# MikeIvanichev/norma

Hardware: AMD Instinct MI355X
Metric: audio-sec/wall-sec (xRT) distil-large-v3 fp16 b32 (higher is better)
Workload: dtype f16

## Files before the change

norma_amd/csrc/k_gemm.hip:

```cpp
#include <stdlib.h>

#include <atomic>

#include "mfma_tile128.h"

#define BM 128
#define BN 128
#define BK 64

__device__ __forceinline__ float gelu_tanh_f(float v) { return gelu_tanh_fast(v); }

__device__ __forceinline__ const half_t *a_row_ptr(const GemmParams &p, int m) {
    if (m >= p.M) m = p.M - 1;
    int b = nh_div(m, p.a_rpb, p.a_magic), r = m - b * p.a_rpb;
    return p.A + (long)b * p.a_bstride + (long)r * p.lda;
}

template <bool SWAP>
__device__ __forceinline__ void gemm_mainloop(const GemmParams &p, char *smem, int m0, int n0, f32x4 (&acc)[4][4]) {
    tile128_mainloop<SWAP>([&](int row) { return a_row_ptr(p, m0 + row); },
                           [&](int row) { return p.W + (long)(n0 + row) * p.K; }, p.K / BK, smem, acc);
}

__device__ __forceinline__ long out_row(const GemmParams &p, int m) {
    int b = nh_div(m, p.o_rpb, p.o_magic), r = m - b * p.o_rpb;
    return (long)b * p.o_bstride + r + p.o_off;
}

__global__ __launch_bounds__(256, 2) void gemm_f16_kernel(GemmParams p) {
    __shared__ __attribute__((aligned(16))) char smem[T128_LDS];
    const int ntn = p.N / BN, ntm = (p.M + BM - 1) / BM;
    const int bid = xcd_contiguous(blockIdx.x, ntn * ntm);
    const int tm = bid / ntn, tn = bid - tm * ntn;
    const int m0 = tm * BM, n0 = tn * BN;
    const int lane = threadIdx.x & 63, w = threadIdx.x >> 6;
    const int wm = w >> 1, wn = w & 1;
    const int fr = lane & 15, fq = lane >> 4;

    f32x4 acc[4][4];
#pragma unroll
    for (int i = 0; i < 4; i++)
#pragma unroll
        for (int j = 0; j < 4; j++) acc[i][j] = (f32x4){0.f, 0.f, 0.f, 0.f};

    const int seg = (p.epi == EPI_F16 || p.epi == EPI_GELU_F16) ? n0 / p.seg_n : 0;
    const bool vt = (p.epi == EPI_F16 && seg == p.vt_seg);
    if (vt) gemm_mainloop<false>(p, smem, m0, n0, acc);
    else gemm_mainloop<true>(p, smem, m0, n0, acc);

    if (vt) {
        half_t *dst = reinterpret_cast<half_t *>(seg == 0 ? p.out[0] : seg == 1 ? p.out[1] : p.out[2]);
#pragma unroll
        for (int i = 0; i < 4; i++) {
            int n = n0 + wn * 64 + 16 * i + fr;
            float bv = p.bias ? p.bias[n] : 0.f;
            int nl = n - seg * p.seg_n, h = nl >> 6, dh = nl & 63;
#pragma unroll
            for (int j = 0; j < 4; j++) {
                int m = m0 + wm * 64 + 16 * j + 4 * fq;
                if (m >= p.M) continue;
                int b = nh_div(m, p.S, p.s_magic), s = m - b * p.S;
                half_t *row = dst + ((long)(b * p.H + h) * NH_DH + dh) * NH_SP;
                if (s + 3 < p.S && m + 3 < p.M) {
                    half4 v = {(half_t)(acc[i][j][0] + bv), (half_t)(acc[i][j][1] + bv),
                               (half_t)(acc[i][j][2] + bv), (half_t)(acc[i][j][3] + bv)};
                    *reinterpret_cast<half4 *>(row + s) = v;
                } else {
                    for (int r = 0; r < 4; r++) {
                        int mm = m + r;
                        if (mm >= p.M) break;
                        int bb = nh_div(mm, p.S, p.s_magic), ss = mm - bb * p.S;
                        dst[((long)(bb * p.H + h) * NH_DH + dh) * NH_SP + ss] = (half_t)(acc[i][j][r] + bv);
                    }
                }
            }
        }
        return;
    }
    half_t *obase = reinterpret_cast<half_t *>(seg == 0 ? p.out[0] : seg == 1 ? p.out[1] : p.out[2]);
#pragma unroll
    for (int i = 0; i < 4; i++) {
        const int n = n0 + wn * 64 + 16 * i + 4 * fq;
        f32x4 bv = {0.f, 0.f, 0.f, 0.f};
        if (p.bias) bv = *reinterpret_cast<const f32x4 *>(p.bias + n);
#pragma unroll
        for (int j = 0; j < 4; j++) {
            const int m = m0 + wm * 64 + 16 * j + fr;
            if (m >= p.M) continue;
            f32x4 v = acc[i][j] + bv;
            if (p.epi == EPI_F16 || p.epi == EPI_GELU_F16) {
                if (p.epi == EPI_F16 && seg == 0 && p.seg0_scale != 0.f) v *= p.seg0_scale;
                if (p.epi == EPI_GELU_F16) {
                    v[0] = gelu_tanh_f(v[0]); v[1] = gelu_tanh_f(v[1]);
                    v[2] = gelu_tanh_f(v[2]); v[3] = gelu_tanh_f(v[3]);
                }
                const int nl = n - seg * p.seg_n;
                half_t *dst = p.head_major ? obase + (((long)nh_div(m, p.S, p.s_magic) * p.H + (nl >> 6)) * p.S + (m - nh_div(m, p.S, p.s_magic) * p.S)) * NH_DH + (nl & 63)
                                           : obase + out_row(p, m) * p.ldo + nl;
                half4 hv = {(half_t)v[0], (half_t)v[1], (half_t)v[2], (half_t)v[3]};
                *reinterpret_cast<half4 *>(dst) = hv;
            } else if (p.epi == EPI_RESID_F32) {
                float *dst = reinterpret_cast<float *>(p.out[0]) + (long)m * p.ldo + n;
                f32x4 x = *reinterpret_cast<const f32x4 *>(dst);
                *reinterpret_cast<f32x4 *>(dst) = x + v;
            } else {
                int s = m - nh_div(m, p.S, p.s_magic) * p.S;
                f32x4 pe = *reinterpret_cast<const f32x4 *>(p.pos + (long)s * p.N + n);
                f32x4 o = {gelu_tanh_f(v[0]) + pe[0], gelu_tanh_f(v[1]) + pe[1], gelu_tanh_f(v[2]) + pe[2],
                           gelu_tanh_f(v[3]) + pe[3]};
                *reinterpret_cast<f32x4 *>(reinterpret_cast<float *>(p.out[0]) + (long)m * p.ldo + n) = o;
            }
        }
    }
}

#define G2_BM 256
#define G2_BN 256
#define G2_GM 4
#define PP_BUF 65536
#define PP_HT 16384
#define PP_RING (2 * PP_BUF)
#define PP_EPI_PITCH 136
#define PP_EPI_WAVE (16 * PP_EPI_PITCH)
#define PP_BIAS (PP_RING + 8 * PP_EPI_WAVE)
#define PP_LDS (PP_BIAS + 2 * 1024)
#define PP_VT_OOB 0xf0000000u

struct PPSource { unsigned ag[2][2], wg[2][2]; };

__device__ __forceinline__ PPSource pp_source(const GemmParams &p, int m0, int n0) {
    int tid = threadIdx.x;
    asm volatile("" : "+v"(tid));
    const int lrow = tid >> 3;
    const int csrc = ((tid & 7) ^ ((lrow >> 1) & 7)) * 8;
    PPSource sg;
#pragma unroll
    for (int h = 0; h < 2; h++)
#pragma unroll
        for (int i = 0; i < 2; i++) {
            const unsigned m = (unsigned)min(m0 + i * 128 + h * 64 + lrow, p.M - 1), b = __umulhi(m, p.a_magic);
            sg.ag[h][i] = b * (unsigned)p.a_bstride + (m - b * (unsigned)p.a_rpb) * (unsigned)p.lda + csrc;
            const int l = lrow + 64 * i;
            sg.wg[h][i] = (unsigned)(n0 + (l >> 5) * 64 + h * 32 + (l & 31)) * (unsigned)p.K + csrc;
        }
    return sg;
}

__device__ __forceinline__ void pp_stage(const GemmParams &p, char *wbase, const PPSource &sg, int t, int which) {
    const int h = (which >> 1) & 1;
    const bool isB = which == 1 || which == 2;
    char *dst = wbase + (t & 1) * PP_BUF + (isB ? 2 * PP_HT : 0) + h * PP_HT;
    const unsigned ko = (unsigned)t * 64u;
    if (isB) {
        __builtin_amdgcn_global_load_lds((gbl_void *)(p.W + (size_t)(sg.wg[h][0] + ko)), (lds_void *)dst, 16, 0, 0);
        __builtin_amdgcn_global_load_lds((gbl_void *)(p.W + (size_t)(sg.wg[h][1] + ko)), (lds_void *)(dst + 8192), 16, 0, 0);
    } else {
        __builtin_amdgcn_global_load_lds((gbl_void *)(p.A + (size_t)(sg.ag[h][0] + ko)), (lds_void *)dst, 16, 0, 0);
        __builtin_amdgcn_global_load_lds((gbl_void *)(p.A + (size_t)(sg.ag[h][1] + ko)), (lds_void *)(dst + 8192), 16, 0, 0);
    }
}

__device__ __forceinline__ void pp_prologue(const GemmParams &p, char *wbase, const PPSource &sg) {
    pp_stage(p, wbase, sg, 0, 0); pp_stage(p, wbase, sg, 0, 1); pp_stage(p, wbase, sg, 0, 2); pp_stage(p, wbase, sg, 0, 3);
    pp_stage(p, wbase, sg, 1, 0); pp_stage(p, wbase, sg, 1, 1);
}

template <bool SWAP>
__device__ __forceinline__ void pp_main(const GemmParams &p, char *smem, char *wbase, const PPSource &sg, f32x4 (&acc)[8][4]) {
    const int lane = threadIdx.x & 63, w = threadIdx.x >> 6;
    const int wr = w >> 2, wc = w & 3;
    const int fr = lane & 15, fq = lane >> 4;
    const int nt = p.K >> 6;
    const int offA0 = (wr * 64 + fr) * 128 + ((fq ^ (fr >> 1)) << 4);
    const int offB0 = (wc * 32 + fr) * 128 + ((fq ^ (fr >> 1)) << 4);
    const char *const pa[2] = {smem + offA0, smem + (offA0 ^ 64)};
    const char *const pb[2] = {smem + offB0, smem + (offB0 ^ 64)};
    half8 fa[4][2], fb[4][2];

#define PP_PHASE(Q, BUF, WAIT, DO_ISSUE, ST)                                                                             \
    {                                                                                                                    \
        constexpr int tb_ = (BUF) * PP_BUF;                                                                              \
        if ((Q) == 0) {                                                                                                  \
            _Pragma("unroll") for (int j = 0; j < 2; j++) _Pragma("unroll") for (int ks = 0; ks < 2; ks++)             \
                fb[j][ks] = *reinterpret_cast<const half8 *>(pb[ks] + (tb_ + 2 * PP_HT + 2048 * j));                    \
            __builtin_amdgcn_sched_barrier(0);                                                                           \
            _Pragma("unroll") for (int i = 0; i < 4; i++) _Pragma("unroll") for (int ks = 0; ks < 2; ks++)             \
                fa[i][ks] = *reinterpret_cast<const half8 *>(pa[ks] + (tb_ + 2048 * i));                               \
        } else if ((Q) == 1) {                                                                                           \
            _Pragma("unroll") for (int j = 0; j < 2; j++) _Pragma("unroll") for (int ks = 0; ks < 2; ks++)             \
                fb[2 + j][ks] = *reinterpret_cast<const half8 *>(pb[ks] + (tb_ + 3 * PP_HT + 2048 * j));                \
        } else if ((Q) == 2) {                                                                                           \
            _Pragma("unroll") for (int i = 0; i < 4; i++) _Pragma("unroll") for (int ks = 0; ks < 2; ks++)             \
                fa[i][ks] = *reinterpret_cast<const half8 *>(pa[ks] + (tb_ + PP_HT + 2048 * i));                       \
        }                                                                                                                \
        __builtin_amdgcn_sched_barrier(0);                                                                               \
        if (DO_ISSUE) pp_stage(p, wbase, sg, (ST), (Q) == 2 ? 0 : (Q) == 3 ? 1 : (Q) == 0 ? 2 : 3);                     \
        if ((WAIT) == 8) asm volatile("s_waitcnt vmcnt(8)" ::: "memory");                                                \
        else if ((WAIT) == 4) asm volatile("s_waitcnt vmcnt(4)" ::: "memory");                                           \
        else if ((WAIT) == 2) asm volatile("s_waitcnt vmcnt(2)" ::: "memory");                                           \
        else if ((WAIT) == 0) asm volatile("s_waitcnt vmcnt(0)" ::: "memory");                                           \
        __builtin_amdgcn_s_barrier();                                                                                    \
        asm volatile("s_waitcnt lgkmcnt(0)" ::: "memory");                                                               \
        __builtin_amdgcn_sched_barrier(0);                                                                               \
        __builtin_amdgcn_s_setprio(1);                                                                                   \
        {                                                                                                                \
            constexpr int ib_ = ((Q) >= 2) ? 4 : 0, jb_ = ((Q) == 1 || (Q) == 2) ? 2 : 0;                                \
            _Pragma("unroll") for (int ks = 0; ks < 2; ks++) _Pragma("unroll") for (int i = 0; i < 4; i++)             \
                _Pragma("unroll") for (int j = 0; j < 2; j++) {                                                         \
                    if (SWAP) acc[ib_ + i][jb_ + j] = __builtin_amdgcn_mfma_f32_16x16x32_f16(fb[jb_ + j][ks], fa[i][ks], acc[ib_ + i][jb_ + j], 0, 0, 0); \
                    else acc[ib_ + i][jb_ + j] = __builtin_amdgcn_mfma_f32_16x16x32_f16(fa[i][ks], fb[jb_ + j][ks], acc[ib_ + i][jb_ + j], 0, 0, 0);      \
                }                                                                                                        \
        }                                                                                                                \
        __builtin_amdgcn_s_setprio(0);                                                                                   \
        __builtin_amdgcn_sched_barrier(0);                                                                               \
        __builtin_amdgcn_s_barrier();                                                                                    \
    }

    asm volatile("s_waitcnt vmcnt(0)" ::: "memory");
    __builtin_amdgcn_s_barrier();
    if (wr == 1) __builtin_amdgcn_s_barrier();
    int t = 0;
    for (; t + 4 <= nt; t += 2) {
        PP_PHASE(0, 0, 8, true, t + 1)
        PP_PHASE(1, 0, 8, true, t + 1)
        PP_PHASE(2, 0, -1, true, t + 2)
        PP_PHASE(3, 0, 8, true, t + 2)
        PP_PHASE(0, 1, 8, true, t + 2)
        PP_PHASE(1, 1, 8, true, t + 2)
        PP_PHASE(2, 1, -1, true, t + 3)
        PP_PHASE(3, 1, 8, true, t + 3)
    }
    PP_PHASE(0, 0, 8, true, t + 1)
    PP_PHASE(1, 0, 8, true, t + 1)
    PP_PHASE(2, 0, -1, false, 0)
    PP_PHASE(3, 0, 4, false, 0)
    PP_PHASE(0, 1, 2, false, 0)
    PP_PHASE(1, 1, 0, false, 0)
    PP_PHASE(2, 1, -1, false, 0)
    PP_PHASE(3, 1, -1, false, 0)
    if (wr == 0) __builtin_amdgcn_s_barrier();
#undef PP_PHASE
}

__device__ __forceinline__ void pp_tile(int vb, int ntn, int ntm, int &tm, int &tn) {
    grouped_tile(xcd_contiguous(vb, ntn * ntm), ntn, ntm, G2_GM, tm, tn);
}


__device__ __forceinline__ void pp_bias_stage(const GemmParams &p, char *smem, int w, int n0, int par) {
    if (!p.bias) return;
    int ln = threadIdx.x;
    asm volatile("" : "+v"(ln));
    __builtin_amdgcn_global_load_lds((gbl_void *)(p.bias + n0 + (w & 3) * 64 + (ln & 63)), (lds_void *)(smem + PP_BIAS + par * 1024 + (w & 3) * 256), 4, 0, 0);
}

__device__ __forceinline__ bool pp_next(const GemmParams &p, char *smem, int w, int par, int &vb, int ntn, int ntm, int &tm, int &tn, PPSource &sg) {
    const int nvb = vb + gridDim.x;
    if (nvb >= ntn * ntm) return false;
    vb = nvb;
    pp_tile(nvb, ntn, ntm, tm, tn);
    pp_bias_stage(p, smem, w, tn * G2_BN, par ^ 1);
    sg = pp_source(p, tm * G2_BM, tn * G2_BN);
    pp_prologue(p, smem + w * 1024, sg);
    return true;
}

__device__ __forceinline__ void pp_row_offsets(const GemmParams &p, int m0, int wm, int ln, unsigned (&off)[16]) {
    const unsigned ml = (unsigned)(m0 + wm * 128 + ((ln >> 3) & 7)), lc = (unsigned)(ln & 7) * 16u;
    const unsigned b0 = __umulhi((unsigned)m0, p.e_magic);
    if (m0 + G2_BM <= p.M && b0 == __umulhi((unsigned)m0 + G2_BM - 1, p.e_magic)) {
        const unsigned base = (b0 * p.e_db + ml) * p.e_rs + lc;
#pragma unroll
        for (int k = 0; k < 16; k++) off[k] = base + (unsigned)(8 * k) * p.e_rs;
    } else {
#pragma unroll
        for (int k = 0; k < 16; k++) {
            const unsigned m = ml + 8 * k;
            off[k] = (__umulhi(m, p.e_magic) * p.e_db + m) * p.e_rs + lc;
        }
    }
}

__device__ __forceinline__ void pp_bias4(const char *smem, int par, int wn, int ln, f32x4 (&bv)[4]) {
    const char *const src = smem + PP_BIAS + par * 1024 + wn * 256 + ((ln >> 4) & 3) * 16;
#pragma unroll
    for (int j = 0; j < 4; j++) bv[j] = *reinterpret_cast<const f32x4 *>(src + 64 * j);
}

template <bool GELU, bool SCALED>
__device__ __forceinline__ void pp_epi_f16(const f32x4 (&acc)[8][4], const f32x4 (&bv)[4], float scale, char *img, int ln,
                                           __amdgpu_buffer_rsrc_t ors, const unsigned (&off)[16]) {
    char *const wr = img + (ln & 15) * PP_EPI_PITCH + ((ln >> 4) & 3) * 8;
    const char *const rd = img + ((ln >> 3) & 7) * PP_EPI_PITCH + (ln & 7) * 16;
#pragma unroll
    for (int i = 0; i < 8; i++) {
#pragma unroll
        for (int j = 0; j < 4; j++) {
            f32x4 v = acc[i][j] + bv[j];
            if (SCALED) v *= scale;
            if (GELU) {
                v[0] = gelu_tanh_f(v[0]); v[1] = gelu_tanh_f(v[1]); v[2] = gelu_tanh_f(v[2]); v[3] = gelu_tanh_f(v[3]);
            }
            half4 hv = {(half_t)v[0], (half_t)v[1], (half_t)v[2], (half_t)v[3]};
            *reinterpret_cast<half4 *>(wr + 32 * j) = hv;
        }
#pragma unroll
        for (int it = 0; it < 2; it++) {
            const half4 lo = *reinterpret_cast<const half4 *>(rd + 8 * it * PP_EPI_PITCH);
            const half4 hi = *reinterpret_cast<const half4 *>(rd + 8 * it * PP_EPI_PITCH + 8);
            const half8 o = {lo[0], lo[1], lo[2], lo[3], hi[0], hi[1], hi[2], hi[3]};
            __builtin_amdgcn_raw_buffer_store_b128(__builtin_bit_cast(u32x4, o), ors, off[2 * i + it], 0, 0);
        }
    }
}

__device__ __forceinline__ void pp_epi_vt(const GemmParams &p, const f32x4 (&acc)[8][4], const float (&bv)[4], char *img, int ln,
                                          half_t *dst, int m0, int wm, int nl0, bool one_clip, unsigned b0) {
    char *const wr = img + (ln & 15) * PP_EPI_PITCH + ((ln >> 4) & 3) * 8;
    const char *const rd = img + ((ln >> 3) & 7) * PP_EPI_PITCH + (ln & 7) * 16;
    const int nl = nl0 + ((ln >> 3) & 7), ml = m0 + wm * 128 + (ln & 7) * 8;
    __amdgpu_buffer_rsrc_t vrs = __builtin_amdgcn_make_buffer_rsrc(dst, 0, (int)p.vt_bytes, 0x00020000);
    const unsigned voff = ((b0 * (unsigned)(p.H * NH_DH) + (unsigned)nl) * NH_SP + ((unsigned)ml - b0 * (unsigned)p.S)) * 2u;
    bool whole[2];
    unsigned wo[2];
    if (!one_clip) {
#pragma unroll
        for (int hh = 0; hh < 2; hh++) {
            const int m = ml + 64 * hh;
            const unsigned b = __umulhi((unsigned)m, p.s_magic), ss = (unsigned)m - b * (unsigned)p.S;
            whole[hh] = (int)ss + 7 < p.S && m + 7 < p.M;
            wo[hh] = ((b * (unsigned)(p.H * NH_DH) + (unsigned)nl) * NH_SP + ss) * 2u;
        }
    }
#pragma unroll
    for (int j = 0; j < 4; j++) {
#pragma unroll
        for (int hh = 0; hh < 2; hh++) {
#pragma unroll
            for (int ii = 0; ii < 4; ii++) {
                const f32x4 a = acc[4 * hh + ii][j];
                half4 v = {(half_t)(a[0] + bv[j]), (half_t)(a[1] + bv[j]), (half_t)(a[2] + bv[j]), (half_t)(a[3] + bv[j])};
                *reinterpret_cast<half4 *>(wr + 32 * ii) = v;
            }
#pragma unroll
            for (int it = 0; it < 2; it++) {
                const half4 lo = *reinterpret_cast<const half4 *>(rd + 8 * it * PP_EPI_PITCH);
                const half4 hi = *reinterpret_cast<const half4 *>(rd + 8 * it * PP_EPI_PITCH + 8);
                if (one_clip) {
                    const half8 o = {lo[0], lo[1], lo[2], lo[3], hi[0], hi[1], hi[2], hi[3]};
                    __builtin_amdgcn_raw_buffer_store_b128(__builtin_bit_cast(u32x4, o), vrs, voff + (unsigned)(((16 * j + 8 * it) * NH_SP + 64 * hh) * 2), 0, 0);
                } else {
                    const unsigned c = (unsigned)((16 * j + 8 * it) * NH_SP * 2);
                    if (whole[hh]) {
                        const half8 o = {lo[0], lo[1], lo[2], lo[3], hi[0], hi[1], hi[2], hi[3]};
                        __builtin_amdgcn_raw_buffer_store_b128(__builtin_bit_cast(u32x4, o), vrs, wo[hh] + c, 0, 0);
                    } else {
#pragma unroll
                        for (int r = 0; r < 8; r++) {
                            const unsigned mm = (unsigned)(ml + 64 * hh + r), bb = __umulhi(mm, p.s_magic);
                            const unsigned eo = (int)mm < p.M ? ((bb * (unsigned)(p.H * NH_DH) + (unsigned)nl) * NH_SP + (mm - bb * (unsigned)p.S)) * 2u : PP_VT_OOB;
                            __builtin_amdgcn_raw_buffer_store_b16(__builtin_bit_cast(short, r < 4 ? lo[r] : hi[r - 4]), vrs, eo + c, 0, 0);
                        }
                    }
                }
            }
        }
    }
}

template <int EPI>
__global__ __launch_bounds__(512) void gemm256_f16_kernel(GemmParams p) {
    __shared__ __attribute__((aligned(16))) char smem[PP_LDS];
    const int ntn = p.N / G2_BN, ntm = (p.M + G2_BM - 1) / G2_BM;
    const int lane = threadIdx.x & 63, w = __builtin_amdgcn_readfirstlane(threadIdx.x >> 6);
    const int wm = w >> 2, wn = w & 3;
    const int fr = lane & 15, fq = lane >> 4;
    char *const wbase = smem + w * 1024;
    char *const img = smem + PP_RING + w * PP_EPI_WAVE;

    int vb = blockIdx.x, tm, tn;
    pp_tile(vb, ntn, ntm, tm, tn);
    if (!p.bias) *reinterpret_cast<float *>(smem + PP_BIAS + threadIdx.x * 4) = 0.f;
    pp_bias_stage(p, smem, w, tn * G2_BN, 0);
    PPSource sg = pp_source(p, tm * G2_BM, tn * G2_BN);
    pp_prologue(p, wbase, sg);
    for (int par = 0;; par ^= 1) {
        const int m0 = tm * G2_BM, n0 = tn * G2_BN;
        f32x4 acc[8][4];
#pragma unroll
        for (int i = 0; i < 8; i++)
#pragma unroll
            for (int j = 0; j < 4; j++) acc[i][j] = (f32x4){0.f, 0.f, 0.f, 0.f};
        if (EPI == EPI_F16 || EPI == EPI_GELU_F16) {
            const int stn = p.seg_n / G2_BN, seg = (tn >= stn) + (tn >= 2 * stn);
            half_t *const ob = reinterpret_cast<half_t *>(seg == 0 ? p.out[0] : seg == 1 ? p.out[1] : p.out[2]);
            const int nl0 = n0 - seg * p.seg_n + wn * 64;
            if (EPI == EPI_F16 && seg == p.vt_seg) {
                pp_main<false>(p, smem, wbase, sg, acc);
                int ln = threadIdx.x;
                asm volatile("" : "+v"(ln));
                const unsigned b0 = __umulhi((unsigned)m0, p.s_magic);
                const bool one_clip = m0 + G2_BM <= p.M && b0 == __umulhi((unsigned)m0 + G2_BM - 1, p.s_magic);
                const bool more = pp_next(p, smem, w, par, vb, ntn, ntm, tm, tn, sg);
                asm volatile("" : "+v"(ln));
                float bv[4];
#pragma unroll
                for (int j = 0; j < 4; j++) bv[j] = *reinterpret_cast<const float *>(smem + PP_BIAS + par * 1024 + wn * 256 + 64 * j + (ln & 15) * 4);
                pp_epi_vt(p, acc, bv, img, ln, ob, m0, wm, nl0, one_clip, b0);
                if (!more) break;
            } else {
                pp_main<true>(p, smem, wbase, sg, acc);
                int ln = threadIdx.x;
                asm volatile("" : "+v"(ln));
                f32x4 bv[4];
                pp_bias4(smem, par, wn, ln, bv);
                const __amdgpu_buffer_rsrc_t ors = __builtin_amdgcn_make_buffer_rsrc(reinterpret_cast<char *>(ob) + p.e_off0 + (long)nl0 * p.e_cs, 0, (int)p.e_bound, 0x00020000);
                unsigned off[16];
                pp_row_offsets(p, m0, wm, ln, off);
                const bool more = pp_next(p, smem, w, par, vb, ntn, ntm, tm, tn, sg);
                if (EPI == EPI_GELU_F16) pp_epi_f16<true, false>(acc, bv, 0.f, img, ln, ors, off);
                else if (seg == 0 && p.seg0_scale != 0.f) pp_epi_f16<false, true>(acc, bv, p.seg0_scale, img, ln, ors, off);
                else pp_epi_f16<false, false>(acc, bv, 0.f, img, ln, ors, off);
                if (!more) break;
            }
            continue;
        }
        pp_main<true>(p, smem, wbase, sg, acc);

        f32x4 rs[4][4];
        __amdgpu_buffer_rsrc_t xrs;
        unsigned xoff = 0;
        if (EPI == EPI_RESID_F32) {
            xrs = __builtin_amdgcn_make_buffer_rsrc(p.out[0], 0, (int)((long)p.M * p.ldo * 4), 0x00020000);
            int ln = threadIdx.x;
            asm volatile("" : "+v"(ln));
            xoff = (unsigned)(((long)(m0 + (ln >> 8) * 128 + (ln & 15)) * p.ldo + n0 + ((ln >> 6) & 3) * 64 + 4 * ((ln >> 4) & 3)) * 4);
#pragma unroll
            for (int ii = 0; ii < 4; ii++)
#pragma unroll
                for (int j = 0; j < 4; j++)
                    rs[ii][j] = __builtin_bit_cast(f32x4, __builtin_amdgcn_raw_buffer_load_b128(xrs, xoff + (unsigned)(64 * ii * p.ldo + 64 * j), 0, 0));
        }
        const bool more = pp_next(p, smem, w, par, vb, ntn, ntm, tm, tn, sg);
        f32x4 bv[4];
        pp_bias4(smem, par, wn, lane, bv);

        if (EPI == EPI_RESID_F32) {
#pragma unroll
            for (int ii = 0; ii < 4; ii++)
#pragma unroll
                for (int j = 0; j < 4; j++)
                    __builtin_amdgcn_raw_buffer_store_b128(__builtin_bit_cast(u32x4, rs[ii][j] + (acc[ii][j] + bv[j])), xrs, xoff + (unsigned)(64 * ii * p.ldo + 64 * j), 0, 0);
#pragma unroll
            for (int ii = 0; ii < 4; ii++)
#pragma unroll
                for (int j = 0; j < 4; j++)
                    rs[ii][j] = __builtin_bit_cast(f32x4, __builtin_amdgcn_raw_buffer_load_b128(xrs, xoff + (unsigned)(64 * (4 + ii) * p.ldo + 64 * j), 0, 0));
#pragma unroll
            for (int ii = 0; ii < 4; ii++)
#pragma unroll
                for (int j = 0; j < 4; j++)
                    __builtin_amdgcn_raw_buffer_store_b128(__builtin_bit_cast(u32x4, rs[ii][j] + (acc[4 + ii][j] + bv[j])), xrs, xoff + (unsigned)(64 * (4 + ii) * p.ldo + 64 * j), 0, 0);
        } else {
#pragma unroll
            for (int j = 0; j < 4; j++) {
                const int n = n0 + wn * 64 + 16 * j + 4 * fq;
#pragma unroll
                for (int i = 0; i < 8; i++) {
                    const int m = m0 + wm * 128 + 16 * i + fr;
                    if (m >= p.M) continue;
                    const f32x4 v = acc[i][j] + bv[j];
                    const int s = m - (int)__umulhi((unsigned)m, p.s_magic) * p.S;
                    const f32x4 pe = *reinterpret_cast<const f32x4 *>(p.pos + (long)s * p.N + n);
                    f32x4 o = {gelu_tanh_f(v[0]) + pe[0], gelu_tanh_f(v[1]) + pe[1], gelu_tanh_f(v[2]) + pe[2],
                               gelu_tanh_f(v[3]) + pe[3]};
                    *reinterpret_cast<f32x4 *>(reinterpret_cast<float *>(p.out[0]) + (long)m * p.ldo + n) = o;
                }
            }
        }
        if (!more) break;
    }
}

static int device_cu_count() {
    static std::atomic<int> cus[NH_MAX_DEVICES];
    int dev = 0;
    if (hipGetDevice(&dev) != hipSuccess || dev < 0 || dev >= NH_MAX_DEVICES) return 256;
    int n = cus[dev].load(std::memory_order_relaxed);
    if (!n) {
        if (hipDeviceGetAttribute(&n, hipDeviceAttributeMultiprocessorCount, dev) != hipSuccess || n <= 0) n = 256;
        cus[dev].store(n, std::memory_order_relaxed);
    }
    return n;
}

static GemmParams with_magics(const GemmParams &p_in) {
    GemmParams p = p_in;
    const long max_m = (long)p.M - 1;
    p.a_magic = nh_magic(p.a_rpb, max_m); p.o_magic = nh_magic(p.o_rpb, max_m); p.s_magic = nh_magic(p.S, max_m);
    return p;
}

static bool plan_gemm256(GemmParams &p) {
    const bool f16 = p.epi == EPI_F16 || p.epi == EPI_GELU_F16;
    if (p.N % G2_BN != 0 || p.K % 128 != 0 || p.M < G2_BM || (f16 && p.seg_n % G2_BN != 0)) return false;
    const unsigned long long lim = 0xffffffffull;
    const long rows = ((long)p.M + G2_BM - 1) / G2_BM * G2_BM;
    if (p.a_magic == ~0u || p.s_magic == ~0u) return false;
    if ((unsigned long long)(p.a_magic ? (p.M - 1) / p.a_rpb : 0) * p.a_bstride + (unsigned long long)p.M * p.lda + p.K > lim) return false;
    if (p.s_magic != 0u) {
        p.s_magic = nh_magic(p.S, rows - 1);
        if (p.s_magic == ~0u) return false;
    }
    if (!f16) return true;
    const bool hm = p.epi == EPI_F16 && p.head_major;
    const long rpb = hm ? p.S : p.o_rpb, bstride = hm ? (long)p.H * p.S : p.o_bstride;
    p.e_rs = hm ? NH_DH * 2 : (unsigned)(p.ldo * 2);
    p.e_cs = hm ? 2L * p.S : 2L;
    p.e_off0 = hm ? 0L : p.o_off * p.ldo * 2;
    p.e_magic = (rpb <= 0 || rpb >= p.M) ? 0u : nh_magic((int)rpb, rows - 1);
    if (p.e_magic == ~0u || (p.e_magic != 0u && bstride < rpb) || p.ldo * 2 > (long)lim || p.e_rs < 128u) return false;
    p.e_db = p.e_magic ? (unsigned)(bstride - rpb) : 0u;
    const unsigned long long last = ((unsigned long long)(p.e_magic ? (p.M - 1) / rpb : 0) * p.e_db + (unsigned long long)(p.M - 1)) * p.e_rs + 128;
    const unsigned long long far = ((unsigned long long)(p.e_magic ? (rows - 1) / rpb : 0) * p.e_db + (unsigned long long)(rows - 1)) * p.e_rs + 128;
    if (far > lim) return false;
    p.e_bound = (unsigned)last;
    if (p.epi == EPI_F16 && p.vt_seg >= 0) {
        if (p.S <= 0) return false;
        const unsigned long long vb = (unsigned long long)((p.M + p.S - 1) / p.S) * p.H * NH_DH * NH_SP * 2;
        if (vb > PP_VT_OOB) return false;
        p.vt_bytes = (unsigned)vb;
    }
    return true;
}

void launch_gemm(const GemmParams &p_in, hipStream_t st) {
    GemmParams p = with_magics(p_in);
    if (plan_gemm256(p)) {
        const int nwg = (p.N / G2_BN) * ((p.M + G2_BM - 1) / G2_BM);
        int cus = p.cus > 0 ? p.cus : device_cu_count();
        cus -= cus % 8;
        const dim3 grid(nwg < cus ? nwg : cus), block(512);
        switch (p.epi) {
            case EPI_F16: hipLaunchKernelGGL(gemm256_f16_kernel<EPI_F16>, grid, block, 0, st, p); break;
            case EPI_GELU_F16: hipLaunchKernelGGL(gemm256_f16_kernel<EPI_GELU_F16>, grid, block, 0, st, p); break;
            case EPI_RESID_F32: hipLaunchKernelGGL(gemm256_f16_kernel<EPI_RESID_F32>, grid, block, 0, st, p); break;
            default: hipLaunchKernelGGL(gemm256_f16_kernel<EPI_CONV2_F32>, grid, block, 0, st, p); break;
        }
        return;
    }
    launch_gemm_128(p, st);
}

void launch_gemm_128(const GemmParams &p_in, hipStream_t st) {
    const GemmParams p = with_magics(p_in);
    int ntn = p.N / BN, ntm = (p.M + BM - 1) / BM;
    hipLaunchKernelGGL(gemm_f16_kernel, dim3(ntn * ntm), dim3(256), 0, st, p);
}
```

Before: 6914.

## Overlap next-tile prologue loads with residual epilogue in persistent GEMM

In the residual-f32 epilogue of the persistent 256-tile GEMM, the next tile's index is computed and its bias and prologue global-to-LDS loads are issued right after the residual loads, before the epilogue stores. pp_main now takes a count of younger outstanding loads, so its initial wait and the first-iteration waits use vmcnt thresholds (48/16, plus a conditional vmcnt(8) skipped at t==0) rather than draining to zero. The aim is to hide next-tile load latency behind epilogue memory traffic. The cost is fragile hand-counted vmcnt bookkeeping and inline-asm buffer loads, which could race if the counts are wrong.

```diff
diff --git a/norma_amd/csrc/k_gemm.hip b/norma_amd/csrc/k_gemm.hip
--- a/norma_amd/csrc/k_gemm.hip
+++ b/norma_amd/csrc/k_gemm.hip
@@ -166,8 +166,10 @@
 }
 
 template <bool SWAP>
-__device__ __forceinline__ void pp_main(const GemmParams &p, char *smem, char *wbase, const PPSource &sg, f32x4 (&acc)[8][4]) {
-    const int lane = threadIdx.x & 63, w = threadIdx.x >> 6;
+__device__ __forceinline__ void pp_main(const GemmParams &p, char *smem, char *wbase, const PPSource &sg, f32x4 (&acc)[8][4], int younger) {
+    int tid = threadIdx.x;
+    asm volatile("" : "+v"(tid));
+    const int lane = tid & 63, w = tid >> 6;
     const int wr = w >> 2, wc = w & 3;
     const int fr = lane & 15, fq = lane >> 4;
     const int nt = p.K >> 6;
@@ -196,6 +198,7 @@
         __builtin_amdgcn_sched_barrier(0);                                                                               \
         if (DO_ISSUE) pp_stage(p, wbase, sg, (ST), (Q) == 2 ? 0 : (Q) == 3 ? 1 : (Q) == 0 ? 2 : 3);                     \
         if ((WAIT) == 8) asm volatile("s_waitcnt vmcnt(8)" ::: "memory");                                                \
+        else if ((WAIT) == 9) asm volatile("s_cmp_eq_u32 %0, 0\n\ts_cbranch_scc1 .Lpp_first%=\n\ts_waitcnt vmcnt(8)\n.Lpp_first%=:" :: "s"(t) : "scc", "memory"); \
         else if ((WAIT) == 4) asm volatile("s_waitcnt vmcnt(4)" ::: "memory");                                           \
         else if ((WAIT) == 2) asm volatile("s_waitcnt vmcnt(2)" ::: "memory");                                           \
         else if ((WAIT) == 0) asm volatile("s_waitcnt vmcnt(0)" ::: "memory");                                           \
@@ -216,15 +219,17 @@
         __builtin_amdgcn_s_barrier();                                                                                    \
     }
 
-    asm volatile("s_waitcnt vmcnt(0)" ::: "memory");
+    if (younger == 48) asm volatile("s_waitcnt vmcnt(48)" ::: "memory");
+    else if (younger == 16) asm volatile("s_waitcnt vmcnt(16)" ::: "memory");
+    else asm volatile("s_waitcnt vmcnt(0)" ::: "memory");
     __builtin_amdgcn_s_barrier();
     if (wr == 1) __builtin_amdgcn_s_barrier();
     int t = 0;
     for (; t + 4 <= nt; t += 2) {
-        PP_PHASE(0, 0, 8, true, t + 1)
-        PP_PHASE(1, 0, 8, true, t + 1)
+        PP_PHASE(0, 0, 9, true, t + 1)
+        PP_PHASE(1, 0, 9, true, t + 1)
         PP_PHASE(2, 0, -1, true, t + 2)
-        PP_PHASE(3, 0, 8, true, t + 2)
+        PP_PHASE(3, 0, 9, true, t + 2)
         PP_PHASE(0, 1, 8, true, t + 2)
         PP_PHASE(1, 1, 8, true, t + 2)
         PP_PHASE(2, 1, -1, true, t + 3)
@@ -263,6 +268,18 @@
     sg = pp_source(p, tm * G2_BM, tn * G2_BN);
     pp_prologue(p, smem + w * 1024, sg);
     return true;
+}
+__device__ __forceinline__ bool pp_next_tile(const GemmParams &p, int &vb, int ntn, int ntm, int &tm, int &tn, PPSource &sg) {
+    const int nvb = vb + gridDim.x;
+    if (nvb >= ntn * ntm) return false;
+    vb = nvb;
+    pp_tile(nvb, ntn, ntm, tm, tn);
+    sg = pp_source(p, tm * G2_BM, tn * G2_BN);
+    return true;
+}
+__device__ __forceinline__ void pp_next_issue(const GemmParams &p, char *smem, int w, int par, int tn, const PPSource &sg) {
+    pp_bias_stage(p, smem, w, tn * G2_BN, par ^ 1);
+    pp_prologue(p, smem + w * 1024, sg);
 }
 
 __device__ __forceinline__ void pp_row_offsets(const GemmParams &p, int m0, int wm, int ln, unsigned (&off)[16]) {
@@ -368,6 +385,24 @@
     }
 }
 
+__device__ __forceinline__ void pp_resid_load(f32x4 (&rs)[4][4], u32x4 xd, unsigned off, unsigned rb) {
+    asm volatile("s_nop 4" ::: "memory");
+#pragma unroll
+    for (int ii = 0; ii < 4; ii++) {
+        const unsigned o = off + (unsigned)ii * rb;
+        asm volatile("buffer_load_dwordx4 %0, %1, %2, 0 offen" : "=v"(rs[ii][0]) : "v"(o), "s"(xd) : "memory");
+        asm volatile("buffer_load_dwordx4 %0, %1, %2, 0 offen offset:64" : "=v"(rs[ii][1]) : "v"(o), "s"(xd) : "memory");
+        asm volatile("buffer_load_dwordx4 %0, %1, %2, 0 offen offset:128" : "=v"(rs[ii][2]) : "v"(o), "s"(xd) : "memory");
+        asm volatile("buffer_load_dwordx4 %0, %1, %2, 0 offen offset:192" : "=v"(rs[ii][3]) : "v"(o), "s"(xd) : "memory");
+    }
+}
+__device__ __forceinline__ void pp_resid_pin(f32x4 (&rs)[4][4]) {
+#pragma unroll
+    for (int ii = 0; ii < 4; ii += 2)
+        asm volatile("" : "+v"(rs[ii][0]), "+v"(rs[ii][1]), "+v"(rs[ii][2]), "+v"(rs[ii][3]), "+v"(rs[ii + 1][0]), "+v"(rs[ii + 1][1]), "+v"(rs[ii + 1][2]), "+v"(rs[ii + 1][3]) :: "memory");
+    __builtin_amdgcn_sched_barrier(0);
+}
+
 template <int EPI>
 __global__ __launch_bounds__(512) void gemm256_f16_kernel(GemmParams p) {
     __shared__ __attribute__((aligned(16))) char smem[PP_LDS];
@@ -384,6 +419,7 @@
     pp_bias_stage(p, smem, w, tn * G2_BN, 0);
     PPSource sg = pp_source(p, tm * G2_BM, tn * G2_BN);
     pp_prologue(p, wbase, sg);
+    int younger = 0;
     for (int par = 0;; par ^= 1) {
         const int m0 = tm * G2_BM, n0 = tn * G2_BN;
         f32x4 acc[8][4];
@@ -396,7 +432,7 @@
             half_t *const ob = reinterpret_cast<half_t *>(seg == 0 ? p.out[0] : seg == 1 ? p.out[1] : p.out[2]);
             const int nl0 = n0 - seg * p.seg_n + wn * 64;
             if (EPI == EPI_F16 && seg == p.vt_seg) {
-                pp_main<false>(p, smem, wbase, sg, acc);
+                pp_main<false>(p, smem, wbase, sg, acc, younger);
                 int ln = threadIdx.x;
                 asm volatile("" : "+v"(ln));
                 const unsigned b0 = __umulhi((unsigned)m0, p.s_magic);
@@ -408,8 +444,9 @@
                 for (int j = 0; j < 4; j++) bv[j] = *reinterpret_cast<const float *>(smem + PP_BIAS + par * 1024 + wn * 256 + 64 * j + (ln & 15) * 4);
                 pp_epi_vt(p, acc, bv, img, ln, ob, m0, wm, nl0, one_clip, b0);
                 if (!more) break;
+                younger = one_clip ? 16 : 0;
             } else {
-                pp_main<true>(p, smem, wbase, sg, acc);
+                pp_main<true>(p, smem, wbase, sg, acc, younger);
                 int ln = threadIdx.x;
                 asm volatile("" : "+v"(ln));
                 f32x4 bv[4];
@@ -422,60 +459,72 @@
                 else if (seg == 0 && p.seg0_scale != 0.f) pp_epi_f16<false, true>(acc, bv, p.seg0_scale, img, ln, ors, off);
                 else pp_epi_f16<false, false>(acc, bv, 0.f, img, ln, ors, off);
                 if (!more) break;
+                younger = 16;
             }
             continue;
         }
-        pp_main<true>(p, smem, wbase, sg, acc);
-
-        f32x4 rs[4][4];
-        __amdgpu_buffer_rsrc_t xrs;
-        unsigned xoff = 0;
+        pp_main<true>(p, smem, wbase, sg, acc, younger);
+
         if (EPI == EPI_RESID_F32) {
-            xrs = __builtin_amdgcn_make_buffer_rsrc(p.out[0], 0, (int)((long)p.M * p.ldo * 4), 0x00020000);
+            const __amdgpu_buffer_rsrc_t xrs = __builtin_amdgcn_make_buffer_rsrc(p.out[0], 0, (int)((long)p.M * p.ldo * 4), 0x00020000);
+            const unsigned long xa = reinterpret_cast<unsigned long>(p.out[0]);
+            const u32x4 xd = {(unsigned)xa, (unsigned)(xa >> 32) & 0xffffu, (unsigned)((long)p.M * p.ldo * 4), 0x00020000u};
             int ln = threadIdx.x;
             asm volatile("" : "+v"(ln));
-            xoff = (unsigned)(((long)(m0 + (ln >> 8) * 128 + (ln & 15)) * p.ldo + n0 + ((ln >> 6) & 3) * 64 + 4 * ((ln >> 4) & 3)) * 4);
+            const unsigned xoff = (unsigned)(((long)(m0 + (ln >> 8) * 128 + (ln & 15)) * p.ldo + n0 + ((ln >> 6) & 3) * 64 + 4 * ((ln >> 4) & 3)) * 4);
+            const unsigned rb = 64u * (unsigned)p.ldo;
+            const bool more = pp_next_tile(p, vb, ntn, ntm, tm, tn, sg);
+            __builtin_amdgcn_sched_barrier(0);
+            f32x4 rs[4][4];
+            pp_resid_load(rs, xd, xoff, rb);
+            if (more) pp_next_issue(p, smem, w, par, tn, sg);
+            if (!more) asm volatile("s_waitcnt vmcnt(0)" ::: "memory");
+            else if (p.bias) asm volatile("s_waitcnt vmcnt(13)" ::: "memory");
+            else asm volatile("s_waitcnt vmcnt(12)" ::: "memory");
+            pp_resid_pin(rs);
+            f32x4 bv[4];
+            pp_bias4(smem, par, wn, ln, bv);
 #pragma unroll
             for (int ii = 0; ii < 4; ii++)
 #pragma unroll
+                for (int j = 0; j < 4; j++) {
+                    acc[ii][j] = rs[ii][j] + (acc[ii][j] + bv[j]);
+                    acc[4 + ii][j] += bv[j];
+                }
+            __builtin_amdgcn_sched_barrier(0);
+            pp_resid_load(rs, xd, xoff + 4u * rb, rb);
+#pragma unroll
+            for (int ii = 0; ii < 4; ii++)
+#pragma unroll
                 for (int j = 0; j < 4; j++)
-                    rs[ii][j] = __builtin_bit_cast(f32x4, __builtin_amdgcn_raw_buffer_load_b128(xrs, xoff + (unsigned)(64 * ii * p.ldo + 64 * j), 0, 0));
+                    __builtin_amdgcn_raw_buffer_store_b128(__builtin_bit_cast(u32x4, acc[ii][j]), xrs, xoff + (unsigned)ii * rb + (unsigned)(64 * j), 0, 0);
+            asm volatile("s_waitcnt vmcnt(16)" ::: "memory");
+            pp_resid_pin(rs);
+#pragma unroll
+            for (int ii = 0; ii < 4; ii++)
+#pragma unroll
+                for (int j = 0; j < 4; j++)
+                    __builtin_amdgcn_raw_buffer_store_b128(__builtin_bit_cast(u32x4, rs[ii][j] + acc[4 + ii][j]), xrs, xoff + (unsigned)(4 + ii) * rb + (unsigned)(64 * j), 0, 0);
+            if (!more) break;
+            younger = 48;
+            continue;
         }
         const bool more = pp_next(p, smem, w, par, vb, ntn, ntm, tm, tn, sg);
         f32x4 bv[4];
         pp_bias4(smem, par, wn, lane, bv);
-
-        if (EPI == EPI_RESID_F32) {
-#pragma unroll
-            for (int ii = 0; ii < 4; ii++)
-#pragma unroll
-                for (int j = 0; j < 4; j++)
-                    __builtin_amdgcn_raw_buffer_store_b128(__builtin_bit_cast(u32x4, rs[ii][j] + (acc[ii][j] + bv[j])), xrs, xoff + (unsigned)(64 * ii * p.ldo + 64 * j), 0, 0);
-#pragma unroll
-            for (int ii = 0; ii < 4; ii++)
-#pragma unroll
-                for (int j = 0; j < 4; j++)
-                    rs[ii][j] = __builtin_bit_cast(f32x4, __builtin_amdgcn_raw_buffer_load_b128(xrs, xoff + (unsigned)(64 * (4 + ii) * p.ldo + 64 * j), 0, 0));
-#pragma unroll
-            for (int ii = 0; ii < 4; ii++)
-#pragma unroll
-                for (int j = 0; j < 4; j++)
-                    __builtin_amdgcn_raw_buffer_store_b128(__builtin_bit_cast(u32x4, rs[ii][j] + (acc[4 + ii][j] + bv[j])), xrs, xoff + (unsigned)(64 * (4 + ii) * p.ldo + 64 * j), 0, 0);
-        } else {
-#pragma unroll
-            for (int j = 0; j < 4; j++) {
-                const int n = n0 + wn * 64 + 16 * j + 4 * fq;
-#pragma unroll
-                for (int i = 0; i < 8; i++) {
-                    const int m = m0 + wm * 128 + 16 * i + fr;
-                    if (m >= p.M) continue;
-                    const f32x4 v = acc[i][j] + bv[j];
-                    const int s = m - (int)__umulhi((unsigned)m, p.s_magic) * p.S;
-                    const f32x4 pe = *reinterpret_cast<const f32x4 *>(p.pos + (long)s * p.N + n);
-                    f32x4 o = {gelu_tanh_f(v[0]) + pe[0], gelu_tanh_f(v[1]) + pe[1], gelu_tanh_f(v[2]) + pe[2],
-                               gelu_tanh_f(v[3]) + pe[3]};
-                    *reinterpret_cast<f32x4 *>(reinterpret_cast<float *>(p.out[0]) + (long)m * p.ldo + n) = o;
-                }
+#pragma unroll
+        for (int j = 0; j < 4; j++) {
+            const int n = n0 + wn * 64 + 16 * j + 4 * fq;
+#pragma unroll
+            for (int i = 0; i < 8; i++) {
+                const int m = m0 + wm * 128 + 16 * i + fr;
+                if (m >= p.M) continue;
+                const f32x4 v = acc[i][j] + bv[j];
+                const int s = m - (int)__umulhi((unsigned)m, p.s_magic) * p.S;
+                const f32x4 pe = *reinterpret_cast<const f32x4 *>(p.pos + (long)s * p.N + n);
+                f32x4 o = {gelu_tanh_f(v[0]) + pe[0], gelu_tanh_f(v[1]) + pe[1], gelu_tanh_f(v[2]) + pe[2],
+                           gelu_tanh_f(v[3]) + pe[3]};
+                *reinterpret_cast<f32x4 *>(reinterpret_cast<float *>(p.out[0]) + (long)m * p.ldo + n) = o;
             }
         }
         if (!more) break;
```

New measurement: 6907 (median of 2 runs). Within noise of the previous version (-0.1%).
